# gitshitou/aclswarm

Hardware: AMD Instinct MI355X
Metric: swarm assignment+control solves/sec (N=100) at 1/2/4/8 MI355X; % HBM roofline (higher is better)
Workload: dtype f64

## Files before the change

aclswarm_amd/csrc/auction.hip:

```cpp
#include <hip/hip_runtime.h>
#include <stdint.h>

#include "../../include/aclswarm_amd.h"
#include "common.h"
#include "control_dev.h"
#include "control_params.h"
#include "neighbourhood_dev.h"
#include "pair_fused.h"
#include "umeyama_dev.h"

namespace acl_amd {

#ifndef ACL_AUCTION_LEVELS
#define ACL_AUCTION_LEVELS 4
#endif
constexpr int kAL = ACL_AUCTION_LEVELS;

__host__ __device__ inline int a16(int x) { return (x + 15) & ~15; }

struct ALayout {
  int C, pq, adjF, items;
  int A, p, qf, out;
  int T, TS;
  int vadj, Pin, Ptin, itm, valid, H, misc, dummy, W1, total;
// ... 72 lines not shown
    load4(pq, j + 7, R3);
  }
}

__device__ __forceinline__ void stamp_phase(const SolveParams& P, int b, int tid, int k) {
  if (P.stamps && tid == 0) P.stamps[(size_t)b * kStampStride + k] = __builtin_amdgcn_s_memtime();
}
__device__ __forceinline__ void stamp_rt(const SolveParams& P, int b, int tid, int k) {
  if (P.stamps && tid == 0) P.stamps[(size_t)b * kStampStride + k] = __builtin_amdgcn_s_memrealtime();
}

#ifndef ACL_AUCTION_PROF
#define ACL_AUCTION_PROF 0
#endif
enum { PS_L0, PS_LV, PS_MB, PS_WALK, PS_SCAN, PS_WB, PS_SEL, PS_BAR, PS_N };
struct SecProf {
  unsigned long long acc[PS_N], last;
  unsigned cols, walks, scans, sels, selx;
  __device__ void start() {
    if (ACL_AUCTION_PROF) {
      for (int k = 0; k < PS_N; ++k) acc[k] = 0;
      cols = walks = scans = sels = selx = 0;
      last = __builtin_amdgcn_s_memtime();
    }
  }
  __device__ void mark(int k) {
    if (ACL_AUCTION_PROF) {
      const unsigned long long t = __builtin_amdgcn_s_memtime();
      acc[k] += t - last;
      last = t;
    }
  }
  __device__ void flush(const SolveParams& P, int b, int lane) {
    if (ACL_AUCTION_PROF && P.stamps && lane == 0) {
      unsigned long long* s = P.stamps + (size_t)b * kStampStride + kStampSec;
      for (int k = 0; k < PS_N; ++k) atomicAdd(s + k, acc[k]);
      atomicAdd(s + PS_N, (unsigned long long)cols | ((unsigned long long)walks << 12) |
                              ((unsigned long long)scans << 24) |
                              ((unsigned long long)sels << 36) | ((unsigned long long)selx << 48));
    }
  }
};

#ifndef ACL_AUCTION_NO_MARGIN
#define ACL_AUCTION_NO_MARGIN 0
#endif
#ifndef ACL_AUCTION_NO_SELMARGIN
#define ACL_AUCTION_NO_SELMARGIN 0
#endif
#ifndef ACL_AUCTION_NO_PUBLISH
#define ACL_AUCTION_NO_PUBLISH 0
#endif

#ifndef ACL_CBAA_COLMAX
#define ACL_CBAA_COLMAX 1
#endif
#ifndef ACL_CBAA_LAZY
#define ACL_CBAA_LAZY 1
#endif

#ifndef ACL_CBAA_WAVES
#define ACL_CBAA_WAVES 8
#endif
#ifndef ACL_PUBLISH_ROUNDS
#define ACL_PUBLISH_ROUNDS 0x7fffffff
#endif

__device__ __forceinline__ float gap_ub(float hi, float lo) {
  const float g = (hi - lo) * __builtin_amdgcn_rcpf(hi) * (1.0f + 0x1p-20f);
  return lo >= 0.5f * hi ? fminf(g, 1.0f) : 1.0f;
}

__device__ __forceinline__ void publish_gap_ub(unsigned long long* margw, const MarginPair& m,
                                               float uhi, float ulo) {
  const float g = fminf(gap_ub(m.hi, m.lo), gap_ub(uhi, ulo));
  const unsigned w = ~wave_max_u32(~__float_as_uint(g));
  if ((threadIdx.x & 63) == 0)
    atomicMin(margw, (unsigned long long)__double_as_longlong((double)__uint_as_float(w)));
}

__device__ __forceinline__ double margin_gap_pair(float hi, float lo) {
  MarginPair m;
  m.hi = hi;
  m.lo = lo;
  return margin_gap(m);
}

__device__ __forceinline__ void margin_track_u(float& hi, float& lo, float h, float l) {
  const bool tie = l == h;
  const bool up = l < h && (double)l * (double)hi > (double)lo * (double)h;
  hi = tie ? 1.0f : (up ? h : hi);
  lo = tie ? 1.0f : (up ? l : lo);
}

enum { FL_OB = 0, FL_DIRTY = 2, FL_CH = 4 };

__device__ __forceinline__ bool lanebit(unsigned long long m) {
  return __builtin_amdgcn_inverse_ballot_w64(m);
}

__device__ __forceinline__ unsigned entry_key(const float* C, int n, int w, int j) {
  return __float_as_uint(C[__umul24(w, n) + j]) + 1u;
}

template <int NC, bool MG>
__device__ __forceinline__ int wave_select(int n, int TS, int v, int lane, const float* C,
                                           const unsigned char* T, bool fresh, MarginPair& m,
                                           unsigned* selx = nullptr) {
  unsigned key[NC];
  float cv[NC], pr[NC];
  bool oth[NC];
  unsigned lm = 0u;
#pragma unroll
  for (int c = 0; c < NC; ++c) {
    const int j = lane + 64 * c;
    const bool ok = j < n;
    const int jj = ok ? j : 0;
    const int w = fresh ? n : T[v * TS + jj];
    cv[c] = C[v * n + jj];
    pr[c] = C[__umul24(w, n) + jj];
    key[c] = (ok && cv[c] > 0.0f && cv[c] > pr[c]) ? __float_as_uint(cv[c]) : 0u;
    oth[c] = ok && w != v;
    lm = lm > key[c] ? lm : key[c];
  }
  const unsigned M = wave_max_u32(lm);
  int js = -1;
  if (M != 0u) {
#pragma unroll
    for (int c = NC - 1; c >= 0; --c) {
      const unsigned long long e = __ballot(key[c] == M);
      if (e) js = 64 * c + __ffsll((long long)e) - 1;
    }
  }
  const float cmax = __uint_as_float(M);
#pragma unroll
  for (int c = 0; c < NC; ++c) {
    if (ACL_AUCTION_PROF && selx) ++*selx;
    if (MG && !ACL_AUCTION_NO_SELMARGIN) {
      const int j = lane + 64 * c;
      const bool isjs = oth[c] && j == js;
      const bool elig = oth[c] && !isjs && key[c] != 0u;
      const bool near = oth[c] && !isjs && key[c] == 0u && cv[c] > 0.0f &&
                        (js < 0 || cv[c] > cmax || (cv[c] == cmax && j < js));
      margin_track_sel(m, isjs ? cv[c] : (elig ? cmax : pr[c]), isjs ? pr[c] : cv[c],
                       isjs || elig || near);
    }
  }
  return js;
}

template <int NC>
__device__ __forceinline__ int first_who(const unsigned long long (&h)[NC], const int (&wu)[NC]) {
  int hl = 0, src = wu[0];
#pragma unroll
  for (int c = NC - 1; c >= 0; --c)
    if (h[c]) {
      hl = __ffsll((long long)h[c]) - 1;
      src = wu[c];
    }
  return __builtin_amdgcn_readlane(src, hl);
}

template <int NC>
__device__ __forceinline__ unsigned level_key(const unsigned (&key)[NC], unsigned cap) {
  unsigned x = 0u;
#pragma unroll
  for (int c = 0; c < NC; ++c) {
    const unsigned y = key[c] < cap ? key[c] : 0u;
    x = x > y ? x : y;
  }
  return wave_max_u32(x);
}

template <int NC>
__device__ __forceinline__ void level_hits(const unsigned long long (&open)[NC],
                                           const unsigned long long (&h)[NC],
                                           const unsigned long long (&vm)[NC][NC],
                                           unsigned long long (&hitm)[NC]) {
#pragma unroll
  for (int c = 0; c < NC; ++c) {
    unsigned long long t = 0ull;
#pragma unroll
    for (int w = 0; w < NC; ++w) t |= vm[c][w] & h[w];
    hitm[c] = __ballot(t != 0ull) & open[c];
  }
}

template <int NC>
__device__ __forceinline__ void level_hits_all(const unsigned long long (&h)[NC],
                                               const unsigned long long (&vm)[NC][NC],
                                               unsigned long long (&hitm)[NC]) {
#pragma unroll
  for (int c = 0; c < NC; ++c) {
    unsigned long long t = 0ull;
#pragma unroll
    for (int w = 0; w < NC; ++w) t |= vm[c][w] & h[w];
    hitm[c] = __ballot(t != 0ull);
  }
}

template <int NC>
__device__ __forceinline__ void runner_up_walk(int n, const unsigned (&key)[NC],
                                               const unsigned (&k1)[NC],
                                               const unsigned long long (&Nd)[NC],
                                               const unsigned long long (&vm)[NC][NC],
// ... 278 lines not shown
  const int tot = __builtin_amdgcn_readfirstlane(off[kAlignS]);
  for (int c0 = 64 * wave; c0 < tot; c0 += 64 * kAlignWaves) {
    const int g = c0 + lane;
    const bool act = g < tot;
    int s = 0;
#pragma unroll
    for (int t = 1; t < kAlignS; ++t) s = off[t] <= g ? t : s;
    int k = g;
#pragma unroll
    for (int t = 1; t < kAlignS; ++t) k = s == t ? g - off[t] : k;
    unsigned long long r[2] = {0ull, 0ull};
    if (act) {
      const int i = (smem + L.items + s * L.its)[k];
      const uint64_t* ga = P.adj + ((size_t)fs[s] * n + i) * NC;
      r[0] = ga[0];
      if (NC > 1) r[1] = ga[NC - 1];
      r[NC - 1] &= lastmask;
      if (i < 64) r[0] |= 1ull << i; else r[1] |= 1ull << (i - 64);
    } else {
      s = 0;
      k = 0;
    }
    const double* pq = reinterpret_cast<const double*>(smem + L.pq + s * L.pqs);
    double* o = reinterpret_cast<double*>(P.ws + P.W.align + (size_t)(bg + s) * P.W.align_stride) +
                6 * k;
    double galign = 1.0;
    align_item<NC>(n, pq, r, act, o, galign);
    if (act) atomicMin(&gapw[s], (unsigned long long)__double_as_longlong(galign));
  }
  __syncthreads();
  if (tid < ns && cnt[tid] > 0) {
    unsigned char* wsa = P.ws + P.W.align + (size_t)(bg + tid) * P.W.align_stride;
    *reinterpret_cast<unsigned long long*>(wsa + itm_off + a16(n)) = gapw[tid];
    *reinterpret_cast<int*>(wsa + itm_off + a16(n) + 8) = cnt[tid];
  }
}

#ifndef ACL_CTL_PRIO
#define ACL_CTL_PRIO 0
#endif
#ifndef ACL_CBAA_PRIO
#define ACL_CBAA_PRIO 0
#endif
#ifndef ACL_AUCTION_OCC_SMALL
#define ACL_AUCTION_OCC_SMALL 6
#endif
template <int NC, int kAB, bool FUSE, bool GM, bool MG>
__global__ void __launch_bounds__(kAB, kAB == 128 ? ACL_AUCTION_OCC_SMALL : 6)
    auction_kernel(const SolveParams P) {
  constexpr int kAW = kAB / 64;
  constexpr int kCW = kAW < ACL_CBAA_WAVES ? kAW : ACL_CBAA_WAVES;
  static_assert((kCW & (kCW - 1)) == 0, "ACL_CBAA_WAVES: a power of two");
  constexpr bool kMarg = MG && !ACL_AUCTION_NO_MARGIN;
  extern __shared__ __attribute__((aligned(16))) unsigned char smem[];
  const int n = P.n;
  const ALayout L = make_alayout(n);
  const int TS = L.TS;
  const int b = P.b0 + blockIdx.x;
  const int tid = threadIdx.x;
  const int lane = tid & 63;
  const int wave = __builtin_amdgcn_readfirstlane(tid >> 6);

  constexpr bool kInlineAlign = kAB <= 256;
  float* C = reinterpret_cast<float*>(smem + L.C);
  double* pq = reinterpret_cast<double*>(smem + L.pq);
  unsigned long long* adjF = reinterpret_cast<unsigned long long*>(smem + L.adjF);
  unsigned char* items = smem + L.items;
  double* p = reinterpret_cast<double*>(smem + L.p);
  double* qf = reinterpret_cast<double*>(smem + L.qf);
  double* out = reinterpret_cast<double*>(smem + L.out);
  unsigned char* T = smem + L.T;
  unsigned long long* vadj = reinterpret_cast<unsigned long long*>(smem + L.vadj);
  unsigned char* Pin = smem + L.Pin;
  unsigned char* Ptin = smem + L.Ptin;
  unsigned char* itm = smem + L.itm;
  unsigned char* validv = smem + L.valid;
  unsigned long long* H = reinterpret_cast<unsigned long long*>(smem + L.H);
  int* misc = reinterpret_cast<int*>(smem + L.misc);
  unsigned long long* margw = reinterpret_cast<unsigned long long*>(misc + M_MARG);
  unsigned long long* W1 = reinterpret_cast<unsigned long long*>(smem + L.W1);
  unsigned* cmax = reinterpret_cast<unsigned*>(smem + L.vadj);

  const int f_in = P.fidx[b];
  const bool fbad = f_in < 0 || f_in >= P.F;
  const int f = fbad ? 0 : f_in;
  const unsigned long long lastmask = (n & 63) ? ((1ull << (n & 63)) - 1ull) : ~0ull;
  const bool rowsm = P.P_rows != nullptr && P.P_rows_on[b] != 0;
  MarginPair mp;
  margin_init(mp);
  stamp_phase(P, b, tid, 0);
  stamp_rt(P, b, tid, kStampRt0);

  const bool hv = tid < n;
  bool pbad = false;
  bool pbig = false;
  unsigned pvr = 0u;
  double qx = 0.0, qy = 0.0, qz = 0.0;
  if (hv) {
    pvr = P.P_in[(size_t)b * n + tid];
    const double* qv = P.q + ((size_t)b * n + tid) * 3;
    qx = qv[0]; qy = qv[1]; qz = qv[2];
  }
  {
    const double* gp = P.p + (size_t)f * n * 3;
    for (int k = tid; k < 3 * n; k += kAB) {
      const double x = gp[k];
      pbad |= !__builtin_isfinite(x);
      if (ACL_PRICE_NANIN) pbig |= !(fabs(x) < 1e100);
      p[k] = x;
      const int j = k / 3, comp = k - 3 * j;
      if (kInlineAlign && comp < 2) pq[4 * j + comp] = x;
    }
    const uint64_t* ga = P.adj + (size_t)f * n * NC;
    for (int k = tid; k < 2 * n; k += kAB) {
      const int i = k >> 1, w = k & 1;
      unsigned long long x = 0ull;
      if (w < NC) {
        x = ga[(size_t)i * NC + w];
        if (w == NC - 1) x &= lastmask;
      }
      adjF[k] = x;
    }
    if (tid < 16) {
      misc[tid] = 0;
      H[tid] = 0ull;
    }
    if (tid < n) W1[tid] = 0ull;
  }
  unsigned long long agap = 0ull;
#ifndef ACL_ALIGN_PREFETCH
#define ACL_ALIGN_PREFETCH 1
#endif
  if (ACL_ALIGN_PREFETCH && !kInlineAlign && !rowsm) {
    const unsigned char* wsa = P.ws + P.W.align + (size_t)b * P.W.align_stride;
    const double* gout = reinterpret_cast<const double*>(wsa);
    for (int k = tid; k < 6 * n; k += kAB) out[k] = gout[k];
    for (int i = tid; i < n; i += kAB) itm[i] = wsa[(size_t)n * 48 + i];
    if (tid == 0) agap = *reinterpret_cast<const unsigned long long*>(wsa + (size_t)n * 48 + a16(n));
  }
  __syncthreads();
  if (tid == 0) {
    misc[M_AGREE] = 1;
    if (fbad) misc[M_BAD] = 1;
    *margw = (unsigned long long)__double_as_longlong(1.0);
  }
  if (__any(pbad) && lane == 0) misc[M_PINF] = 1;
  if (ACL_PRICE_NANIN && __any(pbig) && lane == 0) misc[A_PBIG] = 1;
  if (hv) {
    const int v = tid;
    const unsigned pv = pvr;
    Pin[v] = (unsigned char)pv;
    if (pv >= (unsigned)n) {
      misc[M_BAD] = 1;
    } else {
      const unsigned long long bit = 1ull << (pv & 63);
      if (atomicOr(&H[8 + (pv >> 6)], bit) & bit) misc[M_BAD] = 1;
      Ptin[pv] = (unsigned char)v;
      qf[3 * pv] = qx; qf[3 * pv + 1] = qy; qf[3 * pv + 2] = qz;
      if (kInlineAlign) {
        pq[4 * pv + 2] = qx;
        pq[4 * pv + 3] = qy;
      }
    }
  }
  if (!rowsm) nb_walk_vote<NC>(n, adjF, tid, lane, &misc[M_NBLONG]);
  __syncthreads();
  if (rowsm && !misc[M_BAD]) {
    double galign = 1.0;
    if (hv) {
      const int v = tid, i = Pin[v];
      const uint16_t* row = P.P_rows + ((size_t)b * n + v) * n;
      unsigned long long nbm[2];
      const bool ok = align_own_row<2>(
          n, NC, v, i, adjF + 2 * i, p, [&](int j) { return (int)row[j]; },
          [&](int u, double& x, double& y) {
            x = qf[3 * Pin[u]];
            y = qf[3 * Pin[u] + 1];
          },
          nbm, out + 6 * i, galign);
      if (!ok) misc[M_ROWBAD] = 1;
      vadj[2 * v] = nbm[0];
      vadj[2 * v + 1] = nbm[1];
    }
    for (int i = tid; i < n; i += kAB) itm[i] = (unsigned char)i;
    block_min_gap(margw, galign);
    __syncthreads();
  }
  if (misc[M_BAD] | misc[M_ROWBAD]) {
    for (int v = tid; v < n; v += kAB) {
      P.P_out[(size_t)b * n + v] = P.P_in[(size_t)b * n + v];
      if (P.ca_flag) P.ca_flag[(size_t)b * n + v] = 0;
    }
    for (int k = tid; k < 3 * n; k += kAB) {
      if (P.u) P.u[(size_t)b * n * 3 + k] = 0.0;
      if (P.u_safe) P.u_safe[(size_t)b * n * 3 + k] = 0.0;
    }
    if (P.who)
      for (int k = tid; k < n * n; k += kAB) P.who[(size_t)b * n * n + k] = 0xFFFF;
    if (P.gate_margin && tid == 0) P.gate_margin[b] = __builtin_inf();
    if (tid == 0) {
      acl_swarm_status_t st = {};
      st.flags = ACL_SWARM_BAD_INPUT;
      st.rounds = (uint16_t)(2 * n);
      st.margin = 1.0f;
      P.status[b] = st;
    }
    return;
  }
  if (!rowsm)
    build_neighbourhoods<NC, kAB>(n, adjF, Pin, Ptin, vadj, tid, lane,
                                  __builtin_amdgcn_readfirstlane(misc[M_NBLONG]) == 0);
  if (kInlineAlign && wave == 0 && !rowsm) {
    const int ni = align_worklist<NC>(n, adjF, items, itm, lane);
    if (lane == 0) misc[A_NITEMS] = ni;
  }
  __syncthreads();
  stamp_phase(P, b, tid, 1);
  ACL_AUCTION_STOP_AT(1);

  if (rowsm) {
  } else if constexpr (kInlineAlign) {
    const int nitems = misc[A_NITEMS];
    double galign = 1.0;
    if (wave * 64 < nitems) align_chunk<NC>(n, pq, adjF, items, nitems, wave * 64, lane, out, galign);
    block_min_gap(margw, galign);
  } else if (ACL_ALIGN_PREFETCH) {
    if (tid == 0) atomicMin(margw, agap);
  } else {
    const unsigned char* wsa = P.ws + P.W.align + (size_t)b * P.W.align_stride;
    const int nitems = *reinterpret_cast<const int*>(wsa + (size_t)n * 48 + a16(n) + 8);
    const double* gout = reinterpret_cast<const double*>(wsa);
    for (int k = tid; k < 6 * nitems; k += kAB) out[k] = gout[k];
    for (int i = tid; i < n; i += kAB) itm[i] = wsa[(size_t)n * 48 + i];
    if (tid == 0)
      atomicMin(margw, *reinterpret_cast<const unsigned long long*>(wsa + (size_t)n * 48 + a16(n)));
  }
  __syncthreads();
  stamp_phase(P, b, tid, 2);
  ACL_AUCTION_STOP_AT(2);
  if (P.align_Rt)
    for (int k = tid; k < 6 * n; k += kAB) {
      const int v = k / 6;
      P.align_Rt[(size_t)b * n * 6 + k] = out[6 * itm[Pin[v]] + (k - 6 * v)];
    }

  unsigned* W2 = reinterpret_cast<unsigned*>(C + n * n);
  const int per = kAB / n;
  const int pv = tid % n, j0 = tid / n;
  const bool pact = j0 < per;
  float pbest = 0.0f, psec = 0.0f;
  int pbj = -1;
  {
    int nonfin = 0;
    const bool pfin = misc[M_PINF] == 0;
    const int ip = Pin[pv];
    const double* o = out + 6 * itm[ip];
    const double* qv = qf + 3 * ip;
    const double o0 = o[0], o1 = o[1], o2 = o[2], o3 = o[3], o4 = o[4], o5 = o[5];
    const double q0 = qv[0], q1 = qv[1], q2 = qv[2];
    float* Crow = C + pv * n;
    bool big = !(fabs(o0) < 1e100) || !(fabs(o1) < 1e100) || !(fabs(o2) < 1e100) ||
               !(fabs(o3) < 1e100) || !(fabs(o4) < 1e100) || !(fabs(o5) < 1e100) ||
               !(fabs(q0) < 1e100) || !(fabs(q1) < 1e100) || !(fabs(q2) < 1e100);
    const bool bounded = ACL_PRICE_NANIN && !__any(big) && misc[A_PBIG] == 0;
    auto tasks = [&](auto general) {
      constexpr bool kGen = decltype(general)::value;
      for (int j = j0; pact && j < n; j += per) {
        const double px = p[3 * j], py = p[3 * j + 1], pz = p[3 * j + 2];
        double dx, dy, dz;
        if (!kGen || pfin) {
          dx = q0 - ((o0 * px + o1 * py) + o4);
          dy = q1 - ((o2 * px + o3 * py) + o5);
          dz = q2 - pz;
        } else {
          const double ax = ((o0 * px + o1 * py) + 0.0 * pz) + o4;
          const double ay = ((o2 * px + o3 * py) + 0.0 * pz) + o5;
          const double az = ((0.0 * px + 0.0 * py) + 1.0 * pz) + 0.0;
          dx = q0 - ax; dy = q1 - ay; dz = q2 - az;
        }
        const float c = acl_price((dx * dx + dy * dy) + dz * dz);
        Crow[j] = c;
        if (kGen) nonfin |= (c != c);
        const bool gt = c > pbest;
        psec = gt ? pbest : (c > psec ? c : psec);
        pbj = gt ? j : pbj;
        pbest = gt ? c : pbest;
      }
    };
    if (bounded)
      tasks(std::false_type{});
    else
      tasks(std::true_type{});
    if (pact && pbj >= 0)
      atomicMax(&W1[pv], ((unsigned long long)__float_as_uint(pbest) << 8) |
                             (unsigned long long)(255 - pbj));
    if (__any(nonfin) && lane == 0) misc[M_NONFIN] = 1;
    for (int jj = tid; jj < n; jj += kAB) W2[jj] = 0u;
  }
  unsigned long long vm[NC][NC];
#pragma unroll
  for (int c = 0; c < NC; ++c) {
    const int v = lane + 64 * c;
#pragma unroll
    for (int w = 0; w < NC; ++w) vm[c][w] = (v < n) ? vadj[2 * v + w] : 0ull;
  }
  __syncthreads();
  const bool nonfinite = __builtin_amdgcn_readfirstlane(misc[M_NONFIN]) != 0;
  const unsigned long long nfm = nonfinite ? ~0ull : 0ull;
  stamp_phase(P, b, tid, 3);
  ACL_AUCTION_STOP_AT(3);

  unsigned long long* dmask = H;
  unsigned long long* obm = H + 4;
  {
    const unsigned fill = (unsigned)n * 0x01010101u;
    unsigned* T32 = reinterpret_cast<unsigned*>(T);
    for (int k = tid; k < n * (TS / 4); k += kAB) T32[k] = fill;
    if (ACL_CBAA_COLMAX)
      for (int jj = tid; jj < n; jj += kAB) cmax[jj] = 1u;
    if (pact && pbj >= 0) {
      const int js = 255 - (int)(W1[pv] & 255ull);
      const float cand = pbj == js ? psec : pbest;
      if (cand > 0.0f) atomicMax(&W2[pv], __float_as_uint(cand));
    }
  }
  __syncthreads();
  if (tid < n) {
    const int v = tid;
    const unsigned long long w = W1[v];
    const unsigned sec = W2[v];
    W2[v] = 0u;
    if (w) {
      const int js = 255 - (int)(w & 255ull);
      T[v * TS + js] = (unsigned char)v;
      atomicOr(&dmask[2 + (js >> 6)], 1ull << (js & 63));
      if (ACL_CBAA_COLMAX) atomicMax(&cmax[js], (unsigned)(w >> 8) + 1u);
      if (MG && sec) margin_track(mp, __uint_as_float((unsigned)(w >> 8)), __uint_as_float(sec));
    }
  }
  if (MG && !ACL_AUCTION_NO_PUBLISH) publish_gap_ub(margw, mp, 1.0f, 0.0f);
  __syncthreads();
  ACL_AUCTION_STOP_AT(4);

  if (ACL_CBAA_PRIO) __builtin_amdgcn_s_setprio(ACL_CBAA_PRIO);
  bool okv[NC];
  unsigned long long okm[NC];
  unsigned okk[NC];
  int rowa[NC];
#pragma unroll
  for (int c = 0; c < NC; ++c) {
    okv[c] = lane + 64 * c < n;
    okm[c] = __ballot(okv[c]);
    okk[c] = okv[c] ? 0xFFFFFFFFu : 0u;
    rowa[c] = (okv[c] ? lane + 64 * c : 0) * TS;
  }
  float uhi = 1.0f, ulo = 0.0f;
  int eff = 0;
  unsigned fl = 0u;
  bool evald = false;
  SecProf sp;
  sp.start();
  const int max_rounds = 2 * n;
  for (int r = 1; r <= max_rounds; ++r) {
    const int par = r & 1, npar = par ^ 1;
    const bool cw = wave < kCW;
    unsigned long long mine[NC];
#pragma unroll
    for (int c = 0; c < NC; ++c) mine[c] = 0ull;
    if (cw) {
      int base = 0;
#pragma unroll
      for (int c = 0; c < NC; ++c) {
        const unsigned long long D = uni_u64(dmask[2 * par + c]);
        const int rk = base + (int)__builtin_amdgcn_mbcnt_hi(
                                  (unsigned)(D >> 32), __builtin_amdgcn_mbcnt_lo((unsigned)D, 0u));
        mine[c] = __ballot(((D >> lane) & 1ull) && (rk & (kCW - 1)) == wave);
        base += __popcll(D);
      }
    }
    unsigned long long anymine = 0ull;
#pragma unroll
    for (int c = 0; c < NC; ++c) anymine |= mine[c];
    if (anymine) evald = true;
    if (!ACL_CBAA_LAZY || anymine) {
// ... 495 lines not shown
```

aclswarm_amd/csrc/common.h:

```cpp
#pragma once

#include <hip/hip_runtime.h>
#include <stdint.h>

namespace acl_amd {

constexpr double kPi = 3.14159265358979323846;

template <int CTRL, int RMASK>
__device__ __forceinline__ unsigned dppz(unsigned x) {
  return (unsigned)__builtin_amdgcn_update_dpp(0, (int)x, CTRL, RMASK, 0xF, true);
}

#define ACL_WAVE_REDUCE(x, OP)          \
  x = OP(x, dppz<0xB1, 0xF>(x));        \
  x = OP(x, dppz<0x4E, 0xF>(x));        \
  x = OP(x, dppz<0x124, 0xF>(x));       \
  x = OP(x, dppz<0x128, 0xF>(x));       \
  x = OP(x, dppz<0x142, 0xA>(x));       \
  x = OP(x, dppz<0x143, 0xC>(x))

__device__ __forceinline__ unsigned op_umax(unsigned a, unsigned b) { return a > b ? a : b; }
__device__ __forceinline__ unsigned op_or(unsigned a, unsigned b) { return a | b; }

// ... 269 lines not shown
};

__device__ __forceinline__ double acl_atan_b(double x, const double* tab) {
  const double ax = fabs(x);
  int k = (int)(__float_as_uint((float)ax) >> 21) - (123 << 2) + 1;
  k = k < 0 ? 0 : (k > 33 ? 33 : k);
  const double* rw = tab + 5 * k;
  const double num = __builtin_fma(rw[0], ax, rw[1]);
  const double den = __builtin_fma(rw[2], ax, rw[3]);
  double r = __builtin_amdgcn_rcp(den);
  r = __builtin_fma(__builtin_fma(-den, r, 1.0), r, r);
  const double t = num * r;
  const double z = t * t;
  double p = ACL_MUL_ADD_K(z, -1.0 / 11.0, 1.0 / 9.0);
  p = ACL_FMA_K(z, p, -1.0 / 7.0);
  p = ACL_FMA_K(z, p, 1.0 / 5.0);
  p = ACL_FMA_K(z, p, -1.0 / 3.0);
  const double res = rw[4] + __builtin_fma(t * z, p, t);
  return (ax == __builtin_inf()) ? copysign(1.57079632679489655800e+00, x) : copysign(res, x);
}

__device__ __forceinline__ double acl_atan_b_vote(double x, const double* tab) {
  const double ax = fabs(x);
  int k = (int)(__float_as_uint((float)ax) >> 21) - (123 << 2) + 1;
  asm volatile("" : "+v"(k));
  k = k < 0 ? 0 : (k > 33 ? 33 : k);
  const double* rw = tab + 5 * k;
  const double num = __builtin_fma(rw[0], ax, rw[1]);
  const double den = __builtin_fma(rw[2], ax, rw[3]);
  double r = __builtin_amdgcn_rcp(den);
  r = __builtin_fma(__builtin_fma(-den, r, 1.0), r, r);
  const double t = num * r;
  const double z = t * t;
  double p = ACL_MUL_ADD_K(z, -1.0 / 11.0, 1.0 / 9.0);
  p = ACL_FMA_K(z, p, -1.0 / 7.0);
  p = ACL_FMA_K(z, p, 1.0 / 5.0);
  p = ACL_FMA_K(z, p, -1.0 / 3.0);
  double res = rw[4] + __builtin_fma(t * z, p, t);
  if (__any(ax == __builtin_inf())) {
    unsigned lo, hi;
    asm volatile("v_mov_b32 %0, 0x54442d18\n\tv_mov_b32 %1, 0x3ff921fb" : "=v"(lo), "=v"(hi));
    const double hpi = __longlong_as_double((long long)(((unsigned long long)hi << 32) | lo));
    res = (ax == __builtin_inf()) ? hpi : res;
  }
  return copysign(res, x);
}

#ifndef ACL_PRICE_RSQ
#define ACL_PRICE_RSQ 1
#endif
#ifndef ACL_PRICE_NEWTON
#define ACL_PRICE_NEWTON 1
#endif
__device__ __forceinline__ float acl_price(double x) {
#if ACL_PRICE_RSQ
  double r = __builtin_amdgcn_rsq(x);
  double t = x * r;
  double e = __builtin_fma(-t, r, 1.0);
  r = __builtin_fma(0.5 * r, e, r);
#if ACL_PRICE_NEWTON > 1
  t = x * r;
  e = __builtin_fma(-t, r, 1.0);
  r = __builtin_fma(0.5 * r, e, r);
#endif
  const double d = 1e-8 * r;
  const double y = __builtin_fma(r, __builtin_fma(d, d, -d), r);
  const double lo = 1e-6;
#else
  const double y = div_nr(1.0, sqrt_nr(x) + 1e-8);
  const double lo = 1e-200;
#endif
  const unsigned r29 = (unsigned)((unsigned long long)__double_as_longlong(y) & ((1ull << 29) - 1ull));
  const bool fast = x > lo && x < 1e60 && (r29 - (1u << 28) + 1024u) > 2048u;
  float c = (float)y;
  if (!fast) c = (float)(1.0 / (sqrt(x) + 1e-8));
  return c;
}

__device__ __forceinline__ double wrap_to_pi(double a) {
  if (a > kPi) return a - 2 * kPi;
  if (a < -kPi) return a + 2 * kPi;
  return a;
}

}

namespace acl_amd {

__device__ __forceinline__ int kth_bit(const unsigned long long* m, int NW, int k) {
  for (int w = 0; w < NW; ++w) {
    unsigned long long x = m[w];
    const int pc = __popcll(x);
    if (k < pc) {
      for (int q = 0; q < k; ++q) x &= x - 1;
      return 64 * w + __ffsll((long long)x) - 1;
    }
    k -= pc;
  }
  return -1;
}

__device__ __forceinline__ int wave_ticket(int* misc, int slot, int lane) {
  int t = 0;
  if (lane == 0) t = atomicAdd(&misc[slot], 1);
  return __builtin_amdgcn_readfirstlane(t);
}

struct MarginPair {
  float hi, lo;
};

__device__ __forceinline__ void margin_init(MarginPair& m) {
  m.hi = 1.0f;
  m.lo = 0.0f;
}

__device__ __forceinline__ void margin_track(MarginPair& m, float hi, float lo) {
  if (!(lo < hi)) {
    if (lo == hi) {
      m.hi = 1.0f;
      m.lo = 1.0f;
    }
    return;
  }
  if ((double)lo * (double)m.hi > (double)m.lo * (double)hi) {
    m.hi = hi;
// ... 45 lines not shown
```

aclswarm_amd/csrc/pair_fused.h:

```cpp
#pragma once

#include "control_dev.h"

#ifndef ACL_DIAG_NOPAIR
#define ACL_DIAG_NOPAIR 0
#endif
#ifndef ACL_DIAG_NOLOADS
#define ACL_DIAG_NOLOADS 0
#endif
#ifndef ACL_DIAG_NOLOOP
#define ACL_DIAG_NOLOOP 0
#endif
#ifndef ACL_FUSED_PACK
#define ACL_FUSED_PACK 1
#endif
#ifndef ACL_FUSED_SQRT_VOTE
#define ACL_FUSED_SQRT_VOTE 1
#endif
#ifndef ACL_FUSED_ATAN_VOTE
#define ACL_FUSED_ATAN_VOTE 1
#endif
#if ACL_FUSED_SQRT_VOTE
#define ACL_FUSED_PAIR_E pair_e_vote
#else
#define ACL_FUSED_PAIR_E pair_e
#endif
#if ACL_FUSED_ATAN_VOTE && ACL_GAIN_FASTMATH
#define ACL_FUSED_ATAN acl_atan_b_vote
#else
#define ACL_FUSED_ATAN ACL_GAIN_ATAN
#endif

namespace acl_amd {

struct FusedLayout {
  int pt, adj, etab, rowb, Pt, Pinv, acc, atab, cst, nearb, clf, vel, flags, gmw, caw, total;
};

enum { FC_K1XY, FC_K2XY, FC_K1Z, FC_K2Z, FC_TXY, FC_TZ, FC_WIN, FC_THR2, FC_N };

__host__ __device__ inline FusedLayout make_fused_layout(int n, int kW) {
  const int nb = (n + 7) >> 3, R = 8 * nb;
  FusedLayout L;
  int o = 0;
  L.pt = o;    o = cal16(o + R * 64);
  L.adj = o;   o = cal16(o + R * 2 * 8);
  L.etab = o;  o = cal16(o + R * nb * 4);
  L.rowb = o;  o = cal16(o + (R + 1) * 4);
  L.Pt = o;    o = cal16(o + n * 2);
  L.Pinv = o;  o = cal16(o + n * 2);
  L.acc = o;   o = cal16(o + kW * R * 3 * 8);
  L.atab = o;  o = cal16(o + ACL_ATAB_N * 8);
  L.cst = o;   o = cal16(o + FC_N * 8);
  L.nearb = o; o = cal16(o + 4 * 4);
  L.clf = o;   o = cal16(o + R * 4);
  L.vel = o;   o = cal16(o + n * 24);
  L.flags = o; o = cal16(o + 4);
  L.gmw = o;   o = o + 8;
  L.caw = o;   o = cal16(o + 4);
  L.total = o;
  return L;
}

struct Rec5 {
  double a[5];
};

__device__ __forceinline__ void load_rec5(__amdgpu_buffer_rsrc_t grs, int voff, Rec5& R) {
  const auto r0 = __builtin_amdgcn_raw_buffer_load_b128(grs, voff, 0, 0);
  const auto r1 = __builtin_amdgcn_raw_buffer_load_b128(grs, voff, 16, 0);
  const auto r2 = __builtin_amdgcn_raw_buffer_load_b64(grs, voff, 32, 0);
  __builtin_memcpy(&R.a[0], &r0, 16);
  __builtin_memcpy(&R.a[2], &r1, 16);
// ... 100 lines not shown
  double* qs = acc;

  for (int k = tid; k < ACL_ATAB_N; k += nthreads) atab[k] = ACL_ATAB_AT(k);
  if (GM && tid == 0) gmw = (unsigned long long)__double_as_longlong(__builtin_inf());
  if (tid == 0) {
    *caw = 0u;
    *flags = 0u;
  }
  if (tid < 4) nearb[tid] = 0u;
  for (int k = tid; k < R; k += nthreads) clf[k] = 0u;
  if (tid < FC_N) {
    const double thr_hi = P.s.d_avoid_thresh * (1.0 + 0x1p-40);
    const double v[FC_N] = {P.g.K1_xy, P.g.K2_xy, P.g.K1_z, P.g.K2_z,
                            P.g.e_xy_thr, P.g.e_z_thr, ACL_GATE_WINDOW, thr_hi * thr_hi};
    double x = v[0];
#pragma unroll
    for (int k = 1; k < FC_N; ++k) x = tid == k ? v[k] : x;
    cst[tid] = x;
  }
  {
    bool qbad = false;
    if (tid < n) {
      const int v = tid;
      qs[3 * v] = X.q0;
      qs[3 * v + 1] = X.q1;
      qs[3 * v + 2] = X.q2;
      velv[3 * v] = X.v0;
      velv[3 * v + 1] = X.v1;
      velv[3 * v + 2] = X.v2;
      qbad = !(__builtin_isfinite(X.q0) && __builtin_isfinite(X.q1) && __builtin_isfinite(X.q2));
    }
    if (tid < R) {
      const int i = tid;
      double row[5] = {0.0, 0.0, 0.0, 0.0, 0.0};
      if (i < n) {
        Pinv[Pt[i]] = (uint16_t)i;
        const double x = X.px, y = X.py, z = X.pz;
        row[0] = x;
        row[1] = y;
        row[2] = z;
        row[3] = x * x + y * y;
        row[4] = z * z;
      }
      pt[8 * i + 3] = row[0];
      reinterpret_cast<double4*>(pt + 8 * i)[1] = make_double4(row[1], row[2], row[3], row[4]);
      adjF[2 * i] = X.a0;
      adjF[2 * i + 1] = X.a1;
    }
    if (__any(qbad) && lane == 0) atomicOr(flags, 1u);
  }
  __syncthreads();
  if (tid < R) {
    const int i = tid;
    double q0 = 0.0, q1 = 0.0, q2 = 0.0;
    if (i < n) {
      const int v = Pt[i];
      q0 = qs[3 * v];
      q1 = qs[3 * v + 1];
      q2 = qs[3 * v + 2];
    }
    pt[8 * i] = q0;
    pt[8 * i + 1] = q1;
    pt[8 * i + 2] = q2;
  }
  if (wave == 0) {
    int base = 0;
    for (int i0 = 0; i0 < R; i0 += 64) {
      const int i = i0 + lane;
      const int cnt = (i < R) ? __popcll(adjF[2 * i]) + __popcll(adjF[2 * i + 1]) : 0;
      int x = cnt;
      x += __builtin_amdgcn_update_dpp(0, x, 0x111, 0xF, 0xF, true);
      x += __builtin_amdgcn_update_dpp(0, x, 0x112, 0xF, 0xF, true);
      x += __builtin_amdgcn_update_dpp(0, x, 0x114, 0xF, 0xF, true);
      x += __builtin_amdgcn_update_dpp(0, x, 0x118, 0xF, 0xF, true);
      x += __builtin_amdgcn_update_dpp(0, x, 0x142, 0xA, 0xF, false);
      x += __builtin_amdgcn_update_dpp(0, x, 0x143, 0xC, 0xF, false);
      if (i < R) rowb[i] = base + x - cnt;
      base += __builtin_amdgcn_readlane(x, 63);
    }
    if (lane == 0) rowb[R] = base;
  }
  __syncthreads();
  const unsigned nbm = (65536u + (unsigned)nb - 1u) / (unsigned)nb;
  for (int k = tid; k < R * nb; k += nthreads) {
    const int i = (int)(((unsigned)k * nbm) >> 16), J = k - i * nb;
    const int w = J >> 3, sh = (8 * J) & 63;
    const unsigned long long word = adjF[2 * i + w];
    const unsigned below = (unsigned)__popcll(sh ? (word & ((1ull << sh) - 1ull)) : 0ull) +
                           (w ? (unsigned)__popcll(adjF[2 * i]) : 0u);
    etab[k] = ((unsigned)rowb[i] + below) << 8 | (unsigned)((word >> sh) & 0xFFull);
  }
  for (int k = tid; k < kW * R * 3; k += nthreads) acc[k] = 0.0;
  const bool qfin = (*flags & 1u) == 0u;
  __syncthreads();

  double gmxy = __builtin_inf(), gmz = __builtin_inf();
  if (wave < kW) {
    const int E = __builtin_amdgcn_readfirstlane(rowb[R]);
    const double* G = P.gains + 5 * P.gain_off[f];
    const __amdgpu_buffer_rsrc_t grs =
        __builtin_amdgcn_make_buffer_rsrc((void*)G, (short)0, 5 * E * 8, 0x00020000);
    const int r = lane >> 3, c = lane & 7;
    const int colk = 3 * c + ((lane >> 4) == 0 ? 0 : ((lane >> 4) == 1 ? 2 : 1));
    const bool pack = ACL_FUSED_PACK && (n & 7) >= 1 && (n & 7) <= 4 && nb >= 3;
    const int NR = nb * (nb + 1) / 2 - (pack ? nb - 1 : 0);
    const int NT = NR + (pack ? nb >> 1 : 0);
    const int t0 = (wave * NT) / kW, t1 = ACL_DIAG_NOLOOP ? t0 : ((wave + 1) * NT) / kW;
    const int t1r = t1 < NR ? t1 : NR;
    double* myacc = acc + wave * R * 3;

    int I = 0, J = 0;
    if (t0 < t1r) {
      int rem = t0;
      for (;;) {
        const int len = ((pack && I < nb - 1) ? nb - 1 : nb) - I;
        if (rem < len) break;
        rem -= len;
        ++I;
      }
      J = I + rem;
    }
    auto rec_mask = [&](unsigned x, int s, bool diag, unsigned long long up) {
      return __ballot((x >> s) & 1u) & (diag ? up : ~0ull);
    };
    auto rec_load = [&](unsigned x, int s, unsigned long long m, Rec5& R) {
      const unsigned e = (x >> 8) + (unsigned)__popc(x & ((1u << s) - 1u));
#if ACL_DIAG_NOLOADS
      const double d = (double)(lanebit_u64(m) ? (e & 7u) : 0u) * 0.125;
      R.a[0] = d; R.a[1] = -d; R.a[2] = d; R.a[3] = d; R.a[4] = -d;
#else
      load_rec5(grs, lanebit_u64(m) ? (int)__umul24(e, 40u) : 0x40000000, R);
#endif
    };
    Rec5 X, Y;
    unsigned long long mx = 0ull, my = 0ull;
    if (t0 < t1r) {
      const unsigned xij = etab[__umul24(8 * I + r, nb) + J], xji = etab[__umul24(8 * J + c, nb) + I];
      mx = rec_mask(xij, c, I == J, kTileUpIncl);
      my = rec_mask(xji, r, I == J, kTileUpStrict);
      rec_load(xij, c, mx, X);
      rec_load(xji, r, my, Y);
    }
    double ra0 = 0.0, ra1 = 0.0, ra2 = 0.0;
#pragma unroll 1
    for (int t = t0; t < t1r; ++t) {
#pragma clang fp contract(fast)
      int In = I, Jn = J;
      if (++Jn == ((pack && I < nb - 1) ? nb - 1 : nb)) {
        ++In;
        Jn = In;
      }
      const bool more = t + 1 < t1r;
      unsigned xijn = 0u, xjin = 0u;
      if (more) {
        xijn = etab[__umul24(8 * In + r, nb) + Jn];
        xjin = etab[__umul24(8 * Jn + c, nb) + In];
      }
      const int i = 8 * I + r, j = 8 * J + c;
      const double4* pi = reinterpret_cast<const double4*>(pt + 8 * i);
      const double4* pj = reinterpret_cast<const double4*>(pt + 8 * j);
      const double4 ai = pi[0], aj = pj[0];
      const double q0 = aj.x - ai.x, q1 = aj.y - ai.y, q2 = aj.z - ai.z;
      const double s2 = pair_s2(q0, q1);
      {
        const int nr = n - 8 * I, nc = n - 8 * J;
        const unsigned long long rows = nr >= 8 ? ~0ull : ((1ull << (8 * nr)) - 1ull);
        const unsigned long long cols =
            (nc >= 8 ? 0xFFull : ((1ull << nc) - 1ull)) * 0x0101010101010101ull;
        const unsigned long long vm = rows & cols & (I == J ? kTileUpStrict : ~0ull);
        const unsigned long long nm = __ballot(!(s2 > fcst(cst, FC_THR2))) & vm;
        if (nm) {
          if (lanebit_u64(nm)) {
            atomicOr(&nearb[i >> 5], 1u << (i & 31));
            atomicOr(&nearb[j >> 5], 1u << (j & 31));
          }
        }
      }
      const unsigned long long many = mx | my;
      double Fxy = 0.0, Fz = 0.0;
      if (!ACL_DIAG_NOPAIR && lanebit_u64(many)) {
        const double4 bi = pi[1], bj = pj[1];
        const double pix = ai.w, piy = bi.x, piz = bi.y, pjx = aj.w, pjy = bj.x, pjz = bj.y;
        double e_xy, e_z;
        ACL_FUSED_PAIR_E(q0, q1, q2, bi.z, bj.z, bi.w, bj.w, pix, piy, piz, pjx, pjy, pjz, s2, e_xy,
                         e_z);
        bool gxy, gz;
        gate_decide_t<GM>(fcst(cst, FC_TXY), fcst(cst, FC_TZ), fcst(cst, FC_WIN), e_xy, e_z, q0,
                          q1, q2, bi.z, bj.z, bi.w, bj.w, pix, piy, piz, pjx, pjy, pjz, gxy, gz,
                          gmxy, gmz);
#if ACL_DIAG_NOATAN
        if (gxy) Fxy = fcst(cst, FC_K1XY) * (fcst(cst, FC_K2XY) * e_xy);
        if (gz) Fz = fcst(cst, FC_K1Z) * (fcst(cst, FC_K2Z) * e_z);
#else
        if (gxy) Fxy = fcst(cst, FC_K1XY) * ACL_FUSED_ATAN(fcst(cst, FC_K2XY) * e_xy, atab);
        if (gz) Fz = fcst(cst, FC_K1Z) * ACL_FUSED_ATAN(fcst(cst, FC_K2Z) * e_z, atab);
#endif
      }
      const double f0 = Fxy * q0, f1 = Fxy * q1, f2 = Fz * q2;
      if (lanebit_u64(mx)) {
        if (qfin) {
          ra0 += X.a[1] * q1 + (X.a[0] * q0 + f0);
          ra1 += X.a[3] * q1 + (X.a[2] * q0 + f1);
          ra2 += X.a[4] * q2 + f2;
        } else {
          ra0 += ((X.a[0] * q0 + X.a[1] * q1) + 0.0 * q2) + f0;
          ra1 += ((X.a[2] * q0 + X.a[3] * q1) + 0.0 * q2) + f1;
          ra2 += ((0.0 * q0 + 0.0 * q1) + X.a[4] * q2) + f2;
        }
      }
      unsigned long long mxn = 0ull, myn = 0ull;
      if (more) {
        mxn = rec_mask(xijn, c, In == Jn, kTileUpIncl);
        rec_load(xijn, c, mxn, X);
      }
      double ct0 = 0.0, ct1 = 0.0, ct2 = 0.0;
      if (lanebit_u64(my)) {
        if (qfin) {
          ct0 = Y.a[1] * q1 + (Y.a[0] * q0 + f0);
          ct1 = Y.a[3] * q1 + (Y.a[2] * q0 + f1);
          ct2 = Y.a[4] * q2 + f2;
        } else {
          ct0 = ((Y.a[0] * q0 + Y.a[1] * q1) + 0.0 * q2) + f0;
          ct1 = ((Y.a[2] * q0 + Y.a[3] * q1) + 0.0 * q2) + f1;
          ct2 = ((0.0 * q0 + 0.0 * q1) + Y.a[4] * q2) + f2;
        }
      }
      if (more) {
        myn = rec_mask(xjin, r, In == Jn, kTileUpStrict);
        rec_load(xjin, r, myn, Y);
      }
      {
        const double cs = col3_neg(ct0, ct1, ct2);
        if (lanebit_u64(kColLanes)) unsafeAtomicAdd(myacc + 24 * J + colk, cs);
      }
      if (!more || In != I) {
        ra0 += dpp_f64_all<0xB1>(ra0); ra1 += dpp_f64_all<0xB1>(ra1); ra2 += dpp_f64_all<0xB1>(ra2);
        ra0 += dpp_f64_all<0x4E>(ra0); ra1 += dpp_f64_all<0x4E>(ra1); ra2 += dpp_f64_all<0x4E>(ra2);
        ra0 += dpp_f64_all<0x141>(ra0); ra1 += dpp_f64_all<0x141>(ra1); ra2 += dpp_f64_all<0x141>(ra2);
        if (c == 0) {
          double* a = myacc + 3 * i;
          unsafeAtomicAdd(a, ra0);
          unsafeAtomicAdd(a + 1, ra1);
          unsafeAtomicAdd(a + 2, ra2);
        }
        ra0 = ra1 = ra2 = 0.0;
      }
      I = In;
      J = Jn;
      mx = mxn;
      my = myn;
    }
#pragma unroll 1
    for (int t = t0 > NR ? t0 : NR; t < t1; ++t) {
#pragma clang fp contract(fast)
      const int Ip = 2 * (t - NR);
      const bool two = Ip + 1 < nb - 1;
      const unsigned long long hm = two ? ~0ull : 0x0F0F0F0F0F0F0F0Full;
      const int h = c >> 2, cc = c & 3, Ih = Ip + h;
      const int i = 8 * Ih + r, j = 8 * (nb - 1) + cc;
      const unsigned xij = etab[__umul24(i, nb) + (nb - 1)], xji = etab[__umul24(j, nb) + Ih];
      const unsigned long long pmx = __ballot((xij >> cc) & 1u) & hm;
      const unsigned long long pmy = __ballot((xji >> r) & 1u) & hm;
      rec_load(xij, cc, pmx, X);
      rec_load(xji, r, pmy, Y);
      const double4* pi = reinterpret_cast<const double4*>(pt + 8 * i);
      const double4* pj = reinterpret_cast<const double4*>(pt + 8 * j);
      const double4 ai = pi[0], aj = pj[0];
      const double q0 = aj.x - ai.x, q1 = aj.y - ai.y, q2 = aj.z - ai.z;
      const double s2 = pair_s2(q0, q1);
      {
        const int nc = n - 8 * (nb - 1);
        const unsigned long long vm = (((1ull << nc) - 1ull) * 0x1111111111111111ull) & hm;
        const unsigned long long nm = __ballot(!(s2 > fcst(cst, FC_THR2))) & vm;
        if (nm) {
          if (lanebit_u64(nm)) {
            atomicOr(&nearb[i >> 5], 1u << (i & 31));
            atomicOr(&nearb[j >> 5], 1u << (j & 31));
          }
        }
      }
      double Fxy = 0.0, Fz = 0.0;
      if (!ACL_DIAG_NOPAIR && lanebit_u64(pmx | pmy)) {
        const double4 bi = pi[1], bj = pj[1];
        const double pix = ai.w, piy = bi.x, piz = bi.y, pjx = aj.w, pjy = bj.x, pjz = bj.y;
        double e_xy, e_z;
        ACL_FUSED_PAIR_E(q0, q1, q2, bi.z, bj.z, bi.w, bj.w, pix, piy, piz, pjx, pjy, pjz, s2, e_xy,
                         e_z);
        bool gxy, gz;
        gate_decide_t<GM>(fcst(cst, FC_TXY), fcst(cst, FC_TZ), fcst(cst, FC_WIN), e_xy, e_z, q0,
                          q1, q2, bi.z, bj.z, bi.w, bj.w, pix, piy, piz, pjx, pjy, pjz, gxy, gz,
                          gmxy, gmz);
#if ACL_DIAG_NOATAN
        if (gxy) Fxy = fcst(cst, FC_K1XY) * (fcst(cst, FC_K2XY) * e_xy);
        if (gz) Fz = fcst(cst, FC_K1Z) * (fcst(cst, FC_K2Z) * e_z);
#else
        if (gxy) Fxy = fcst(cst, FC_K1XY) * ACL_FUSED_ATAN(fcst(cst, FC_K2XY) * e_xy, atab);
        if (gz) Fz = fcst(cst, FC_K1Z) * ACL_FUSED_ATAN(fcst(cst, FC_K2Z) * e_z, atab);
#endif
      }
      const double f0 = Fxy * q0, f1 = Fxy * q1, f2 = Fz * q2;
      double pa0 = 0.0, pa1 = 0.0, pa2 = 0.0;
      if (lanebit_u64(pmx)) {
        if (qfin) {
          pa0 = X.a[1] * q1 + (X.a[0] * q0 + f0);
          pa1 = X.a[3] * q1 + (X.a[2] * q0 + f1);
          pa2 = X.a[4] * q2 + f2;
        } else {
          pa0 = ((X.a[0] * q0 + X.a[1] * q1) + 0.0 * q2) + f0;
          pa1 = ((X.a[2] * q0 + X.a[3] * q1) + 0.0 * q2) + f1;
          pa2 = ((0.0 * q0 + 0.0 * q1) + X.a[4] * q2) + f2;
        }
      }
      double ct0 = 0.0, ct1 = 0.0, ct2 = 0.0;
      if (lanebit_u64(pmy)) {
        if (qfin) {
          ct0 = Y.a[1] * q1 + (Y.a[0] * q0 + f0);
          ct1 = Y.a[3] * q1 + (Y.a[2] * q0 + f1);
          ct2 = Y.a[4] * q2 + f2;
        } else {
          ct0 = ((Y.a[0] * q0 + Y.a[1] * q1) + 0.0 * q2) + f0;
          ct1 = ((Y.a[2] * q0 + Y.a[3] * q1) + 0.0 * q2) + f1;
          ct2 = ((0.0 * q0 + 0.0 * q1) + Y.a[4] * q2) + f2;
        }
      }
      {
// ... 89 lines not shown
```

Baseline: 8.479 million.

## Trim second-best tracking, simplify first_who, price range check, and padded-row masks

Several independent micro-optimisations. When margins are disabled, the auction skips second-best price tracking and the prefetched alignment-gap read. first_who now uses unconditional readlanes with selects instead of a branchy scan. acl_price replaces double-precision range compares with an integer compare on the high word. Padding rows are placed far away (2^500 offsets) so the pair kernel can drop its validity masks, and the next-tile record loads are made unconditional to keep them in scalar registers. The far-padding trick depends on the distance threshold never accepting padded pairs, and the high-word range check changes the bounds slightly.

```diff
diff --git a/aclswarm_amd/csrc/auction.hip b/aclswarm_amd/csrc/auction.hip
--- a/aclswarm_amd/csrc/auction.hip
+++ b/aclswarm_amd/csrc/auction.hip
@@ -148,6 +148,13 @@
 #define ACL_AUCTION_NO_PUBLISH 0
 #endif
 
+#ifndef ACL_START_LEAN
+#define ACL_START_LEAN 1
+#endif
+#ifndef ACL_FIRST_WHO_RL
+#define ACL_FIRST_WHO_RL 1
+#endif
+
 #ifndef ACL_CBAA_COLMAX
 #define ACL_CBAA_COLMAX 1
 #endif
@@ -247,6 +254,15 @@
 
 template <int NC>
 __device__ __forceinline__ int first_who(const unsigned long long (&h)[NC], const int (&wu)[NC]) {
+#if ACL_FIRST_WHO_RL
+  int who = __builtin_amdgcn_readlane(wu[NC - 1], (__ffsll((long long)h[NC - 1]) - 1) & 63);
+#pragma unroll
+  for (int c = NC - 2; c >= 0; --c) {
+    const int x = __builtin_amdgcn_readlane(wu[c], (__ffsll((long long)h[c]) - 1) & 63);
+    who = h[c] ? x : who;
+  }
+  return who;
+#endif
   int hl = 0, src = wu[0];
 #pragma unroll
   for (int c = NC - 1; c >= 0; --c)
@@ -631,6 +647,7 @@
   constexpr int kCW = kAW < ACL_CBAA_WAVES ? kAW : ACL_CBAA_WAVES;
   static_assert((kCW & (kCW - 1)) == 0, "ACL_CBAA_WAVES: a power of two");
   constexpr bool kMarg = MG && !ACL_AUCTION_NO_MARGIN;
+  constexpr bool kSec = MG || !ACL_START_LEAN;
   extern __shared__ __attribute__((aligned(16))) unsigned char smem[];
   const int n = P.n;
   const ALayout L = make_alayout(n);
@@ -715,7 +732,8 @@
     const double* gout = reinterpret_cast<const double*>(wsa);
     for (int k = tid; k < 6 * n; k += kAB) out[k] = gout[k];
     for (int i = tid; i < n; i += kAB) itm[i] = wsa[(size_t)n * 48 + i];
-    if (tid == 0) agap = *reinterpret_cast<const unsigned long long*>(wsa + (size_t)n * 48 + a16(n));
+    if (kSec && tid == 0)
+      agap = *reinterpret_cast<const unsigned long long*>(wsa + (size_t)n * 48 + a16(n));
   }
   __syncthreads();
   if (tid == 0) {
@@ -804,7 +822,7 @@
     if (wave * 64 < nitems) align_chunk<NC>(n, pq, adjF, items, nitems, wave * 64, lane, out, galign);
     block_min_gap(margw, galign);
   } else if (ACL_ALIGN_PREFETCH) {
-    if (tid == 0) atomicMin(margw, agap);
+    if (kSec && tid == 0) atomicMin(margw, agap);
   } else {
     const unsigned char* wsa = P.ws + P.W.align + (size_t)b * P.W.align_stride;
     const int nitems = *reinterpret_cast<const int*>(wsa + (size_t)n * 48 + a16(n) + 8);
@@ -861,7 +879,7 @@
         Crow[j] = c;
         if (kGen) nonfin |= (c != c);
         const bool gt = c > pbest;
-        psec = gt ? pbest : (c > psec ? c : psec);
+        if (kSec) psec = gt ? pbest : (c > psec ? c : psec);
         pbj = gt ? j : pbj;
         pbest = gt ? c : pbest;
       }
@@ -897,7 +915,7 @@
     for (int k = tid; k < n * (TS / 4); k += kAB) T32[k] = fill;
     if (ACL_CBAA_COLMAX)
       for (int jj = tid; jj < n; jj += kAB) cmax[jj] = 1u;
-    if (pact && pbj >= 0) {
+    if (kSec && pact && pbj >= 0) {
       const int js = 255 - (int)(W1[pv] & 255ull);
       const float cand = pbj == js ? psec : pbest;
       if (cand > 0.0f) atomicMax(&W2[pv], __float_as_uint(cand));
@@ -907,8 +925,11 @@
   if (tid < n) {
     const int v = tid;
     const unsigned long long w = W1[v];
-    const unsigned sec = W2[v];
-    W2[v] = 0u;
+    unsigned sec = 0u;
+    if (kSec) {
+      sec = W2[v];
+      W2[v] = 0u;
+    }
     if (w) {
       const int js = 255 - (int)(w & 255ull);
       T[v * TS + js] = (unsigned char)v;
diff --git a/aclswarm_amd/csrc/common.h b/aclswarm_amd/csrc/common.h
--- a/aclswarm_amd/csrc/common.h
+++ b/aclswarm_amd/csrc/common.h
@@ -345,6 +345,10 @@
 #ifndef ACL_PRICE_NEWTON
 #define ACL_PRICE_NEWTON 1
 #endif
+#ifndef ACL_PRICE_HIWORD
+#define ACL_PRICE_HIWORD 1
+#endif
+constexpr unsigned kPriceHiLo = 0x3EB0C6F8u, kPriceHiHi = 0x4C63E9E4u;
 __device__ __forceinline__ float acl_price(double x) {
 #if ACL_PRICE_RSQ
   double r = __builtin_amdgcn_rsq(x);
@@ -364,7 +368,13 @@
   const double lo = 1e-200;
 #endif
   const unsigned r29 = (unsigned)((unsigned long long)__double_as_longlong(y) & ((1ull << 29) - 1ull));
+#if ACL_PRICE_RSQ && ACL_PRICE_HIWORD
+  const unsigned xh = (unsigned)((unsigned long long)__double_as_longlong(x) >> 32);
+  const bool fast = xh - kPriceHiLo < kPriceHiHi - kPriceHiLo && (r29 - (1u << 28) + 1024u) > 2048u;
+  (void)lo;
+#else
   const bool fast = x > lo && x < 1e60 && (r29 - (1u << 28) + 1024u) > 2048u;
+#endif
   float c = (float)y;
   if (!fast) c = (float)(1.0 / (sqrt(x) + 1e-8));
   return c;
diff --git a/aclswarm_amd/csrc/pair_fused.h b/aclswarm_amd/csrc/pair_fused.h
--- a/aclswarm_amd/csrc/pair_fused.h
+++ b/aclswarm_amd/csrc/pair_fused.h
@@ -19,6 +19,12 @@
 #endif
 #ifndef ACL_FUSED_ATAN_VOTE
 #define ACL_FUSED_ATAN_VOTE 1
+#endif
+#ifndef ACL_FUSED_FARPAD
+#define ACL_FUSED_FARPAD 1
+#endif
+#ifndef ACL_FUSED_MORE_SGPR
+#define ACL_FUSED_MORE_SGPR 1
 #endif
 #if ACL_FUSED_SQRT_VOTE
 #define ACL_FUSED_PAIR_E pair_e_vote
@@ -225,7 +231,7 @@
   __syncthreads();
   if (tid < R) {
     const int i = tid;
-    double q0 = 0.0, q1 = 0.0, q2 = 0.0;
+    double q0 = ACL_FUSED_FARPAD ? 0x1p500 * (double)(i - n + 1) : 0.0, q1 = 0.0, q2 = 0.0;
     if (i < n) {
       const int v = Pt[i];
       q0 = qs[3 * v];
@@ -324,6 +330,7 @@
         Jn = In;
       }
       const bool more = t + 1 < t1r;
+      constexpr bool kPre = ACL_FUSED_MORE_SGPR != 0 && !GM;
       unsigned xijn = 0u, xjin = 0u;
       if (more) {
         xijn = etab[__umul24(8 * In + r, nb) + Jn];
@@ -336,11 +343,15 @@
       const double q0 = aj.x - ai.x, q1 = aj.y - ai.y, q2 = aj.z - ai.z;
       const double s2 = pair_s2(q0, q1);
       {
+#if ACL_FUSED_FARPAD
+        const unsigned long long vm = I == J ? kTileUpStrict : ~0ull;
+#else
         const int nr = n - 8 * I, nc = n - 8 * J;
         const unsigned long long rows = nr >= 8 ? ~0ull : ((1ull << (8 * nr)) - 1ull);
         const unsigned long long cols =
             (nc >= 8 ? 0xFFull : ((1ull << nc) - 1ull)) * 0x0101010101010101ull;
         const unsigned long long vm = rows & cols & (I == J ? kTileUpStrict : ~0ull);
+#endif
         const unsigned long long nm = __ballot(!(s2 > fcst(cst, FC_THR2))) & vm;
         if (nm) {
           if (lanebit_u64(nm)) {
@@ -382,7 +393,7 @@
         }
       }
       unsigned long long mxn = 0ull, myn = 0ull;
-      if (more) {
+      if (kPre || more) {
         mxn = rec_mask(xijn, c, In == Jn, kTileUpIncl);
         rec_load(xijn, c, mxn, X);
       }
@@ -398,7 +409,7 @@
           ct2 = ((0.0 * q0 + 0.0 * q1) + Y.a[4] * q2) + f2;
         }
       }
-      if (more) {
+      if (kPre || more) {
         myn = rec_mask(xjin, r, In == Jn, kTileUpStrict);
         rec_load(xjin, r, myn, Y);
       }
@@ -442,8 +453,12 @@
       const double q0 = aj.x - ai.x, q1 = aj.y - ai.y, q2 = aj.z - ai.z;
       const double s2 = pair_s2(q0, q1);
       {
+#if ACL_FUSED_FARPAD
+        const unsigned long long vm = hm;
+#else
         const int nc = n - 8 * (nb - 1);
         const unsigned long long vm = (((1ull << nc) - 1ull) * 0x1111111111111111ull) & hm;
+#endif
         const unsigned long long nm = __ballot(!(s2 > fcst(cst, FC_THR2))) & vm;
         if (nm) {
           if (lanebit_u64(nm)) {
```

Result: faster. 8.815 million (median of 6 runs) (+4.0%).
